# tensorflow/recommenders

Measured on NVIDIA H100. Metric: queries/sec brute-force top-K (1Mx64 candidates), higher is better.
Workload: dtype f32 (fp16 wgmma screening, fp32 accumulate + exact fp32 re-scoring)

## Files before the change

### recommenders_b200/csrc/rowselect.cuh

```cuda
#pragma once
#include "common.cuh"
#include <limits.h>

namespace tfrs {

constexpr int RS_THREADS = 256;

__device__ __forceinline__ void bitonic_sort_desc(float* bs, long long* bi, int P) {
  for (int size = 2; size <= P; size <<= 1) {
    for (int stride = size >> 1; stride > 0; stride >>= 1) {
      for (int t = threadIdx.x; t < (P >> 1); t += blockDim.x) {
        int lo = 2 * t - (t & (stride - 1));
        int hi = lo + stride;
        bool desc = ((lo & size) == 0);
        float sl = bs[lo], sh = bs[hi];
        long long il = bi[lo], ih = bi[hi];
        bool hi_better = better(sh, ih, sl, il);
        bool lo_better = better(sl, il, sh, ih);
        if (desc ? hi_better : lo_better) { bs[lo] = sh; bs[hi] = sl; bi[lo] = ih; bi[hi] = il; }
      }
      __syncthreads();
    }
  }
}

static inline int pow2_ceil(int x) { int p = 1; while (p < x) p <<= 1; return p; }
static inline int rowselect_cap(int k) { int c = pow2_ceil(2 * k); return c < 1024 ? 1024 : c; }
static inline size_t rowselect_smem(int cap, size_t extra) { return (size_t)cap * 12 + extra; }

template <class Provider>
__global__ void __launch_bounds__(RS_THREADS)
row_topk_kernel(Provider prov, int k, int cap, float* __restrict__ out_s, long long* __restrict__ out_i,
                int out_ld) {
  extern __shared__ __align__(16) unsigned char rs_smem[];
  long long* bi = reinterpret_cast<long long*>(rs_smem);
  float* bs = reinterpret_cast<float*>(rs_smem + (size_t)cap * 8);
  void* extra = rs_smem + (size_t)cap * 12;
  __shared__ int cnt_sh;
  __shared__ float thr_s_sh;
  __shared__ long long thr_i_sh;
  __shared__ int full_sh;

  const int row = blockIdx.x;
  const int tid = threadIdx.x;
  if (tid == 0) { cnt_sh = 0; full_sh = 0; thr_s_sh = 0.f; thr_i_sh = 0; }
  prov.begin(row, extra);
  __syncthreads();

  const long long total = prov.count(row);
  const int min_room = cap / 4;
  long long pos = 0;
  while (pos < total) {
    __syncthreads();
    const int cnt0 = cnt_sh;
    const bool full = full_sh != 0;
    const float ts = thr_s_sh;
    const long long ti = thr_i_sh;
    __syncthreads();
    const int slab = (int)min((long long)(cap - cnt0), total - pos);
    for (int t = tid; t < slab; t += RS_THREADS) {
      float s; long long i;
      prov.get(row, pos + t, s, i);
      if (!full || better(s, i, ts, ti)) {
        int p = atomicAdd(&cnt_sh, 1);
        bs[p] = s; bi[p] = i;
      }
    }
    __syncthreads();
    pos += slab;
    const int cnt = cnt_sh;
    if (pos < total && cap - cnt >= min_room) continue;
    int P = 2; while (P < cnt) P <<= 1;
    for (int t = cnt + tid; t < P; t += RS_THREADS) { bs[t] = -INFINITY; bi[t] = LLONG_MAX; }
    __syncthreads();
    if (cnt > 1) bitonic_sort_desc(bs, bi, P);
    if (tid == 0) {
      int keep = cnt < k ? cnt : k;
      cnt_sh = keep;
      if (keep == k) { full_sh = 1; thr_s_sh = bs[k - 1]; thr_i_sh = bi[k - 1]; }
    }
  }
  __syncthreads();
  const int n_out = cnt_sh;
  for (int t = tid; t < n_out; t += RS_THREADS) {
    out_s[(long long)row * out_ld + t] = bs[t];
    out_i[(long long)row * out_ld + t] = bi[t];
  }
}

}
```

### recommenders_b200/csrc/topk_tc.cu

```cuda
#include <cuda_fp16.h>
#include <math.h>
#include <stdlib.h>
#include <type_traits>
#include "rowselect.cuh"
#include "tc_ptx.cuh"

namespace tfrs {
namespace tc {

constexpr int TILE_N = 128;
constexpr int TILE_M = 128;
constexpr int QBLK = 256;
constexpr int KSLAB = 64;
constexpr int SLAB_BYTES = TILE_N * 128;
constexpr int HEADER_BYTES = 1024;
constexpr int THREADS = 512;
constexpr int CONSUMER_WARPS = 16;
constexpr int CAND_CAP = 2048;
constexpr int MAX_SAMPLE_STRIDE = 4;
constexpr int FIN_MAX_PARTS = 2 * 132;
constexpr int MAX_BINS = 1024;
constexpr int FP16_TARGET = 15;
constexpr float E_REL = 0.00108f;
constexpr float E_ACC = 0.00013f;
// ... 380 lines not shown
}
__device__ __forceinline__ unsigned int warp_kth_largest_smem(const unsigned int* keys, int n, int k, int lane, unsigned int prefix, int top_bit) {
  for (int bit = top_bit; bit >= 0; --bit) {
    const unsigned int cand = prefix | (1u << bit);
    int c = 0;
    for (int t = lane; t < n; t += 32) c += (keys[t] >= cand) ? 1 : 0;
    c = __reduce_add_sync(0xffffffffu, c);
    if (c >= k) prefix = cand;
  }
  return prefix;
}

template <int KPL>
__global__ void __launch_bounds__(256)
tc_threshold_kernel(const float* __restrict__ binmax, int bins_ld, int n_bins, int k, const float* __restrict__ margin,
                    float* __restrict__ thr, unsigned int* __restrict__ overflow, long long Q) {
  const int lane = threadIdx.x & 31;
  const long long row = ((long long)blockIdx.x * 256 + threadIdx.x) >> 5;
  if (row >= Q) return;
  const float* src = binmax + row * bins_ld;
  unsigned int key[KPL];
#pragma unroll
  for (int j = 0; j < KPL; ++j) { const int i = j * 32 + lane; key[j] = i < n_bins ? f2key(__ldg(src + i)) : 0u; }
  const unsigned int kth = warp_kth_largest_regs<KPL>(key, k);
  if (lane == 0) { thr[row] = key2f(kth) - margin[row]; overflow[row] = 0; }
}

enum { FIN_TOPK = 0, FIN_EXCLUDE = 1, FIN_COUNT = 2 };
constexpr int FW_WARPS = 4;

struct FinParams {
  const float* q; const float* corpus; int d; int k; long long index_offset; long long N; long long Q;
  const unsigned int* count; const float* cand_s; const unsigned int* cand_i; int segs; int cap_part;
  const float* cut; const float* thr; unsigned int* overflow;
  int cap_keys, cap_band;
  unsigned int* band_idx; int* band_n;
  int allow_short;
  float* out_s; long long* out_i;
  const long long* identifiers; const long long* exclusions; int n_excl; int k_out;
  const float* pos; const int* qexp; const IndexHeader* hdr; int* out_count;
};

__device__ __forceinline__ float exact_score(const float* __restrict__ qs, const float* __restrict__ c, int d) {
  float acc = 0.f;
  if ((d & 31) == 0) {
    for (int kk = 0; kk < d; kk += 32) {
      float4 cv[8];
#pragma unroll
      for (int u = 0; u < 8; ++u) cv[u] = __ldg(reinterpret_cast<const float4*>(c + kk) + u);
#pragma unroll
      for (int u = 0; u < 8; ++u) {
// ... 49 lines not shown
    akey[t] = ((unsigned long long)f2key(adj) << 32) | (unsigned long long)(0xFFFFFFFFu - (unsigned int)t);
  }
  __syncwarp();
  for (int t = lane; t < kf; t += 32) {
    const unsigned long long mine = akey[t];
    int rank = 0;
    for (int j = 0; j < kf; ++j) rank += (akey[j] > mine) ? 1 : 0;
    if (rank < p.k_out) {
      const unsigned long long e = srt[t];
      p.out_s[row * p.k_out + rank] = rank_key_score(e);
      p.out_i[row * p.k_out + rank] = (long long)rank_key_index(e) + p.index_offset;
    }
  }
}

__host__ __device__ inline size_t sel_warp_bytes(int cap_keys, int segs) {
  return (size_t)cap_keys * 4 + (size_t)cap_keys * 2 + (size_t)((segs + 1 + 3) & ~3) * 4;
}
constexpr int SEL_WARPS = 8;

__device__ __forceinline__ bool load_record(const FinParams& p, long long row, const int* soff, int rec, int total_rec,
                                            unsigned int& ix0, float (&sc)[8]) {
  if (rec >= total_rec) return false;
  int lo = 0, hi = p.segs;
  while (hi - lo > 1) { const int mid = (lo + hi) >> 1; if (soff[mid] <= rec) lo = mid; else hi = mid; }
  const long long at = (row * p.segs + lo) * p.cap_part + (rec - soff[lo]);
  ix0 = __ldg(p.cand_i + at);
  const float4 s0 = __ldg(reinterpret_cast<const float4*>(p.cand_s + at * 8));
  const float4 s1 = __ldg(reinterpret_cast<const float4*>(p.cand_s + at * 8) + 1);
  sc[0] = s0.x; sc[1] = s0.y; sc[2] = s0.z; sc[3] = s0.w; sc[4] = s1.x; sc[5] = s1.y; sc[6] = s1.z; sc[7] = s1.w;
  return true;
}

template <int MODE>
__global__ void __launch_bounds__(SEL_WARPS * 32)
tc_select_kernel(const FinParams p) {
  extern __shared__ __align__(16) unsigned char fsm[];
  const int warp = threadIdx.x >> 5, lane = threadIdx.x & 31;
  const long long row = (long long)blockIdx.x * SEL_WARPS + warp;
  if (row >= p.Q) return;
  unsigned char* base = fsm + (size_t)warp * sel_warp_bytes(p.cap_keys, p.segs);
  unsigned int* keys = reinterpret_cast<unsigned int*>(base);
  unsigned short* loc = reinterpret_cast<unsigned short*>(keys + p.cap_keys);
  int* soff = reinterpret_cast<int*>(loc + p.cap_keys);
  const unsigned int n32 = (unsigned int)p.N;
  unsigned int* band = p.band_idx + row * p.cap_band;

  int carry = 0; bool bad = false;
  for (int s0 = 0; s0 < p.segs; s0 += 32) {
    const int s = s0 + lane;
    int c = 0;
    if (s < p.segs) {
      const unsigned int cc = __ldg(p.count + row * p.segs + s);
      if (cc > (unsigned int)p.cap_part) bad = true; else c = (int)cc;
    }
    const int inc = warp_incl_scan(c, lane);
    if (s < p.segs) soff[s + 1] = carry + inc;
    carry += __shfl_sync(0xffffffffu, inc, 31);
  }
  if (lane == 0) soff[0] = 0;
  if (__any_sync(0xffffffffu, bad)) {
    if (lane == 0) { p.overflow[row] = 1; p.band_n[row] = 0; }
    return;
  }
  __syncwarp();
  const int total_rec = soff[p.segs];
  const float thr_row = p.thr[row];
  if (MODE != FIN_COUNT && total_rec >= 8192) {
    if (lane == 0) { p.overflow[row] = 1; p.band_n[row] = 0; }
    return;
  }

  if (MODE == FIN_COUNT) {
    const float eps = 0.5f * p.cut[row];
    const float pos_s = ldexpf(p.pos[row], p.hdr->st.exp + p.qexp[row]);
    const float hi = pos_s + eps, lo_b = pos_s - eps;
    int definite = 0, m = 0;
    for (int rb = 0; rb < total_rec; rb += 32) {
      unsigned int ix0 = 0, amb = 0; int cnt = 0; float sc[8];
      if (load_record(p, row, soff, rb + lane, total_rec, ix0, sc)) {
#pragma unroll
        for (int j = 0; j < 8; ++j) {
          const bool real = ix0 + j < n32;
          definite += (real && sc[j] > hi) ? 1 : 0;
          const bool a = real && sc[j] > lo_b && !(sc[j] > hi);
          amb |= a ? (1u << j) : 0u; cnt += a ? 1 : 0;
        }
      }
      const int incl = warp_incl_scan(cnt, lane);
      const int tot = __shfl_sync(0xffffffffu, incl, 31);
      if (m + tot <= p.cap_band) {
        int at_pos = m + incl - cnt;
#pragma unroll
        for (int j = 0; j < 8; ++j)
          if (amb & (1u << j)) { band[at_pos] = ix0 + j; ++at_pos; }
      }
      m += tot;
    }
    definite = __reduce_add_sync(0xffffffffu, definite);
    if (lane == 0) {
      if (definite >= p.k) { p.out_count[row] = p.k; p.band_n[row] = 0; p.overflow[row] = 0; }
      else if (m > p.cap_band) { p.overflow[row] = 1; p.band_n[row] = 0; }
      else { p.out_count[row] = definite; p.band_n[row] = m; p.overflow[row] = 0; }
    }
    return;
  }

  int n = 0;
  unsigned int kmax = 0u, kmin = 0xFFFFFFFFu;
  for (int rb = 0; rb < total_rec; rb += 32) {
    float sc[8]; unsigned int ix0 = 0, keep = 0; int cnt = 0;
    if (load_record(p, row, soff, rb + lane, total_rec, ix0, sc)) {
#pragma unroll
      for (int j = 0; j < 8; ++j) {
        const bool kp = sc[j] >= thr_row && ix0 + j < n32;
        keep |= kp ? (1u << j) : 0u; cnt += kp ? 1 : 0;
      }
    }
    const int incl = warp_incl_scan(cnt, lane);
    const int tot = __shfl_sync(0xffffffffu, incl, 31);
    if (n + tot <= p.cap_keys) {
      int at_pos = n + incl - cnt;
#pragma unroll
      for (int j = 0; j < 8; ++j) {
        if (keep & (1u << j)) {
          const unsigned int key = f2key(sc[j] + 0.0f);
          kmax = max(kmax, key); kmin = min(kmin, key);
          keys[at_pos] = key;
          loc[at_pos] = (unsigned short)(((rb + lane) << 3) | j);
          ++at_pos;
        }
      }
    }
    n += tot;
  }
  if (n > p.cap_keys || (n < p.k && !p.allow_short)) { if (lane == 0) { p.overflow[row] = 1; p.band_n[row] = 0; } return; }
  __syncwarp();
  if (n < p.k) {
    const bool fits = n <= p.cap_band;
    for (int t = lane; t < n && fits; t += 32) {
      const unsigned int l = loc[t];
      const int rec = (int)(l >> 3);
      int lo = 0, hi = p.segs;
      while (hi - lo > 1) { const int mid = (lo + hi) >> 1; if (soff[mid] <= rec) lo = mid; else hi = mid; }
      band[t] = __ldg(p.cand_i + (row * p.segs + lo) * p.cap_part + (rec - soff[lo])) + (l & 7u);
    }
    if (lane == 0) { p.overflow[row] = fits ? 0u : 1u; p.band_n[row] = fits ? n : 0; }
    return;
  }
  kmax = __reduce_max_sync(0xffffffffu, kmax); kmin = __reduce_min_sync(0xffffffffu, kmin);
  unsigned int tau_key;
  {
    const unsigned int diff = kmax ^ kmin;
    const int top = diff ? (31 - __clz(diff)) : -1;
    const unsigned int prefix0 = top >= 31 ? 0u : (top < 0 ? kmax : (kmax & ~((2u << top) - 1u)));
    if (n <= 512) {
      unsigned int kr[16];
#pragma unroll
      for (int j = 0; j < 16; ++j) { const int t = j * 32 + lane; kr[j] = t < n ? keys[t] : 0u; }
      tau_key = warp_kth_largest_regs<16>(kr, p.k, prefix0, top);
    } else if (n <= 1024) {
      unsigned int kr[32];
#pragma unroll
      for (int j = 0; j < 32; ++j) { const int t = j * 32 + lane; kr[j] = t < n ? keys[t] : 0u; }
      tau_key = warp_kth_largest_regs<32>(kr, p.k, prefix0, top);
    } else {
      tau_key = warp_kth_largest_smem(keys, n, p.k, lane, prefix0, top);
    }
  }
  const float lim = key2f(tau_key) - p.cut[row];
  if (!p.allow_short && (!(lim >= thr_row) || !(lim > -INFINITY))) { if (lane == 0) { p.overflow[row] = 1; p.band_n[row] = 0; } return; }
  const unsigned int lim_key = f2key(lim + 0.0f);
  const unsigned int lt_mask = (1u << lane) - 1u;
  int m = 0;
  for (int tb = 0; tb < n; tb += 32) {
    const int t = tb + lane;
    const bool kp = t < n && keys[t] >= lim_key;
    const unsigned int vote = __ballot_sync(0xffffffffu, kp);
    if (kp) {
      const int at_pos = m + __popc(vote & lt_mask);
      if (at_pos < p.cap_band) {
        const unsigned int l = loc[t];
        const int rec = (int)(l >> 3);
        int lo = 0, hi = p.segs;
        while (hi - lo > 1) { const int mid = (lo + hi) >> 1; if (soff[mid] <= rec) lo = mid; else hi = mid; }
        band[at_pos] = __ldg(p.cand_i + (row * p.segs + lo) * p.cap_part + (rec - soff[lo])) + (l & 7u);
      }
    }
    m += __popc(vote);
  }
  if (lane == 0) {
    if (m > p.cap_band) { p.overflow[row] = 1; p.band_n[row] = 0; }
    else { p.overflow[row] = 0; p.band_n[row] = m; }
  }
}

constexpr int RS_BLOCK = 128;
template <int MODE>
__global__ void __launch_bounds__(RS_BLOCK)
tc_rescore_kernel(const FinParams p) {
  extern __shared__ __align__(16) unsigned char rsm[];
  unsigned long long* sk = reinterpret_cast<unsigned long long*>(rsm);
  float* qs = reinterpret_cast<float*>(sk + p.cap_band);
  unsigned long long* srt = reinterpret_cast<unsigned long long*>(qs + ((p.d + 3) & ~3));
  __shared__ int greater_sh;
  const long long row = blockIdx.x;
  const int tid = threadIdx.x;
  if (p.overflow[row] != 0) return;
  const int m = p.band_n[row];
  if (MODE == FIN_COUNT && m == 0) return;
  for (int t = tid; t < p.d; t += RS_BLOCK) qs[t] = p.q[row * p.d + t];
  if (tid == 0) greater_sh = 0;
  __syncthreads();
  const unsigned int* band = p.band_idx + row * p.cap_band;
  if (MODE == FIN_COUNT) {
    const float pos = p.pos[row];
    int g = 0;
    for (int t = tid; t < m; t += RS_BLOCK) g += (exact_score(qs, p.corpus + (long long)band[t] * p.d, p.d) > pos) ? 1 : 0;
    g = __reduce_add_sync(0xffffffffu, g);
    if ((tid & 31) == 0 && g) atomicAdd(&greater_sh, g);
    __syncthreads();
    if (tid == 0) { const int c = p.out_count[row] + greater_sh; p.out_count[row] = c < p.k ? c : p.k; }
    return;
  }
  if (p.d == 64) {
    constexpr int RPB = RS_BLOCK / 8;
    constexpr int MAXR = 8;
    const int sub = tid & 7, grp = tid >> 3;
    for (int t0 = 0; t0 < m; t0 += RPB * MAXR) {
      float4 a[MAXR], b[MAXR];
#pragma unroll
      for (int r = 0; r < MAXR; ++r) {
        const int t = t0 + r * RPB + grp;
        if (t < m) {
          const float4* src = reinterpret_cast<const float4*>(p.corpus + (long long)band[t] * 64) + sub * 2;
          a[r] = __ldg(src); b[r] = __ldg(src + 1);
        }
      }
      const float q0 = qs[sub * 8], q1 = qs[sub * 8 + 1], q2 = qs[sub * 8 + 2], q3 = qs[sub * 8 + 3];
      const float q4 = qs[sub * 8 + 4], q5 = qs[sub * 8 + 5], q6 = qs[sub * 8 + 6], q7 = qs[sub * 8 + 7];
#pragma unroll
      for (int r = 0; r < MAXR; ++r) {
        const int t = t0 + r * RPB + grp;
        const bool live = t < m;
        float acc = 0.f;
#pragma unroll
        for (int step = 0; step < 8; ++step) {
          if (sub == step && live) {
            acc = fmaf(q0, a[r].x, acc); acc = fmaf(q1, a[r].y, acc); acc = fmaf(q2, a[r].z, acc); acc = fmaf(q3, a[r].w, acc);
            acc = fmaf(q4, b[r].x, acc); acc = fmaf(q5, b[r].y, acc); acc = fmaf(q6, b[r].z, acc); acc = fmaf(q7, b[r].w, acc);
          }
          acc = __shfl_sync(0xffffffffu, acc, (threadIdx.x & 24) | step);
        }
        if (live && sub == 0) sk[t] = rank_key(acc, band[t]);
      }
    }
  } else {
    for (int t = tid; t < m; t += RS_BLOCK) {
      const unsigned int idx = band[t];
      sk[t] = rank_key(exact_score(qs, p.corpus + (long long)idx * p.d, p.d), idx);
    }
  }
  __syncthreads();
  if (MODE == FIN_TOPK && m < p.k)
    for (int t = m + tid; t < p.k; t += RS_BLOCK) { p.out_s[row * p.k + t] = -INFINITY; p.out_i[row * p.k + t] = LLONG_MAX; }
  for (int t = tid; t < m; t += RS_BLOCK) {
    const unsigned long long mine = sk[t];
    int rank = 0;
#pragma unroll 4
    for (int j = 0; j < m; ++j) rank += (sk[j] > mine) ? 1 : 0;
    if (rank < p.k) {
      if (MODE == FIN_TOPK) {
        p.out_s[row * p.k + rank] = rank_key_score(mine);
        p.out_i[row * p.k + rank] = (long long)rank_key_index(mine) + p.index_offset;
      } else {
        srt[rank] = mine;
      }
    }
  }
  if (MODE == FIN_EXCLUDE) {
    __syncthreads();
// ... 22 lines not shown
  __device__ void begin(int row, void* extra) {
    qs = reinterpret_cast<float*>(extra);
    if (overflow[row] != 0) for (int t = threadIdx.x; t < d; t += blockDim.x) qs[t] = q[(long long)row * d + t];
  }
  __device__ long long count(int row) const { return overflow[row] != 0 ? N : 0; }
  __device__ void get(int, long long t, float& s, long long& i) const {
    const float* c = corpus + t * d;
    float acc = 0.f;
    for (int kk = 0; kk < d; ++kk) acc = fmaf(qs[kk], __ldg(c + kk), acc);
    s = acc; i = index_offset + t;
  }
};

__global__ void __launch_bounds__(256)
tc_count_fallback_kernel(const float* __restrict__ q, const float* __restrict__ corpus, long long N, int d, int k,
                         const float* __restrict__ pos, const unsigned int* __restrict__ overflow, int* __restrict__ out_count) {
  __shared__ float qs[128];
  __shared__ int total;
  const int row = blockIdx.x;
  if (overflow[row] == 0) return;
  for (int t = threadIdx.x; t < d; t += 256) qs[t] = q[(long long)row * d + t];
  if (threadIdx.x == 0) total = 0;
  __syncthreads();
  const float ps = pos[row];
  int c = 0;
  for (long long t = threadIdx.x; t < N; t += 256) {
    const float* cr = corpus + t * d;
    float acc = 0.f;
    for (int kk = 0; kk < d; ++kk) acc = fmaf(qs[kk], __ldg(cr + kk), acc);
    c += (acc + 0.0f > ps) ? 1 : 0;
  }
  c = __reduce_add_sync(0xffffffffu, c);
  if ((threadIdx.x & 31) == 0) atomicAdd(&total, c);
  __syncthreads();
  if (threadIdx.x == 0) out_count[row] = total < k ? total : k;
}

struct Prof {
  bool on = false;
  static constexpr int MAXC = 512, STAGES_ = 4;
  cudaEvent_t ev[MAXC][STAGES_ + 1];
  int created = 0, calls = 0;
};
static Prof g_prof;
static void prof_mark(cudaStream_t st, int stage) {
  if (!g_prof.on || g_prof.calls >= Prof::MAXC) return;
  int c = g_prof.calls;
  while (g_prof.created <= c) {
    for (int s = 0; s <= Prof::STAGES_; ++s) cudaEventCreate(&g_prof.ev[g_prof.created][s]);
    ++g_prof.created;
  }
  cudaEventRecord(g_prof.ev[c][stage], st);
  if (stage == Prof::STAGES_) ++g_prof.calls;
}

struct Plan {
  int kb, stages; long long n_tiles; int nqb; long long Qp;
  int stride, n_sample, group, bins_per_part, n_bins, bins_ld, parts_sample, parts_full, cap_part, cap_keys, cap_band;
  size_t smem;
  size_t o_qimg, o_margin, o_cut, o_thr, o_qexp, o_count, o_ovf, o_binmax, o_cand, o_tmp, o_band, o_bandn, total;
};

static bool make_plan(long long Q, long long N, int d, int k, Plan& pl) {
  if (d <= 0 || d > 128 || Q <= 0 || N <= 0 || k <= 0) return false;
  pl.kb = (d + KSLAB - 1) / KSLAB;
  pl.stages = pl.kb == 1 ? 6 : 4;
  pl.n_tiles = ceil_div(N, TILE_N);
  pl.nqb = (int)ceil_div(Q, QBLK);
  pl.Qp = (long long)pl.nqb * QBLK;
  if (k > 256 || N >= (1ll << 31)) return false;
  const long long full_tiles = N / TILE_N;
  if (full_tiles < 1) return false;
  pl.stride = MAX_SAMPLE_STRIDE;
#ifdef TFRS_DEBUG_SWITCHES
  { static int ov = getenv("TFRS_TC_SAMPLE_STRIDE") ? atoi(getenv("TFRS_TC_SAMPLE_STRIDE")) : 0; if (ov >= 1 && ov <= 16) pl.stride = ov; }
// ... 26 lines not shown
    pl.cap_band = ck / 2;
  }
  pl.smem = (size_t)(2 + pl.stages) * pl.kb * SLAB_BYTES + 1024  + 256 ;
  size_t o = 0;
  auto take = [&](size_t bytes) { size_t r = o; o += align_up(bytes, 1024); return r; };
  pl.o_qimg = take((size_t)pl.nqb * 2 * pl.kb * SLAB_BYTES);
  pl.o_margin = take((size_t)pl.Qp * 4);
  pl.o_cut = take((size_t)pl.Qp * 4);
  pl.o_thr = take((size_t)pl.Qp * 4);
  pl.o_qexp = take((size_t)pl.Qp * 4);
  pl.o_count = take((size_t)pl.Qp * pl.parts_full * 2 * 4);
  pl.o_ovf = take((size_t)pl.Qp * 4);
  pl.o_binmax = take((size_t)pl.Qp * pl.bins_ld * 4);
  pl.o_cand = take((size_t)pl.Qp * pl.parts_full * 2 * pl.cap_part * (8 * 4 + 4));
  pl.o_tmp = take((size_t)Q * k * 12);
  pl.o_band = take((size_t)pl.Qp * pl.cap_band * 4);
  pl.o_bandn = take((size_t)pl.Qp * 4);
  pl.total = o;
  return true;
}

template <int KB, int STAGES>
static int launch_scans(const Plan& pl, ScanParams sp, cudaStream_t st, int mode) {
  auto ks = tc_scan_kernel<KB, STAGES, MODE_SAMPLE>;
  auto kf = tc_scan_kernel<KB, STAGES, MODE_FILTER>;
  TFRS_DYN_SMEM(ks, (int)pl.smem);
  TFRS_DYN_SMEM(kf, (int)pl.smem);
  if (mode == MODE_SAMPLE) {
    sp.parts = pl.parts_sample; sp.n_seq = pl.n_sample; sp.stride = pl.stride;
    ks<<<(unsigned)(pl.nqb * sp.parts), THREADS, pl.smem, st>>>(sp);
  } else {
    sp.parts = pl.parts_full; sp.n_seq = (int)pl.n_tiles; sp.stride = 1;
    kf<<<(unsigned)(pl.nqb * sp.parts), THREADS, pl.smem, st>>>(sp);
  }
  TFRS_LAUNCH_CHECK();
  return TFRS_OK;
}

static int launch_scan_mode(const Plan& pl, const ScanParams& sp, cudaStream_t st, int mode) {
  if (pl.kb == 1) return launch_scans<1, 6>(pl, sp, st, mode);
  return launch_scans<2, 4>(pl, sp, st, mode);
}

template <int MODE>
static int launch_finalize(FinParams fp, cudaStream_t st) {
  auto ksel = tc_select_kernel<MODE>;
  auto krs = tc_rescore_kernel<MODE>;
  TFRS_DYN_SMEM(ksel, (int)(SEL_WARPS * sel_warp_bytes(4096, FIN_MAX_PARTS)));
  ksel<<<(unsigned)ceil_div(fp.Q, SEL_WARPS), SEL_WARPS * 32, SEL_WARPS * sel_warp_bytes(fp.cap_keys, fp.segs), st>>>(fp);
  TFRS_LAUNCH_CHECK();
  const size_t rs_smem = (size_t)fp.cap_band * 8 + (size_t)((fp.d + 3) & ~3) * 4 + (MODE == FIN_EXCLUDE ? (size_t)fp.k * 16 : 0);
  TFRS_DYN_SMEM(krs, 64 * 1024);
  krs<<<(unsigned)fp.Q, RS_BLOCK, rs_smem, st>>>(fp);
  TFRS_LAUNCH_CHECK();
  return TFRS_OK;
}

struct Call {
  int mode;
  const float* q; long long Q; const float* corpus; const void* index_buf; long long N; int d; int k; long long index_offset;
  void* ws; size_t ws_bytes; cudaStream_t st;
  float* out_s; long long* out_i;
  const long long* identifiers; const long long* exclusions; int n_excl; int k_out;
  const float* pos; int* out_count;
  ThrHook hook; void* hook_ctx; int allow_short;
};

static int run_call(const Call& c) {
// ... 6 lines not shown
  if (!c.ws || c.ws_bytes < pl.total + 16) { set_error("topk_tc: workspace too small (%zu < %zu)", c.ws_bytes, pl.total + 16); return TFRS_ERR_WORKSPACE_TOO_SMALL; }
  cudaStream_t st = c.st;
  unsigned char* w = (unsigned char*)(((uintptr_t)c.ws + 15) & ~(uintptr_t)15);
  unsigned char* qimg = w + pl.o_qimg;
  float* margin = (float*)(w + pl.o_margin);
  float* cut = (float*)(w + pl.o_cut);
  float* thr = (float*)(w + pl.o_thr);
  int* qexp = (int*)(w + pl.o_qexp);
  unsigned int* count = (unsigned int*)(w + pl.o_count);
  unsigned int* ovf = (unsigned int*)(w + pl.o_ovf);
  float* binmax = (float*)(w + pl.o_binmax);
  float* cand_s = (float*)(w + pl.o_cand);
  unsigned int* cand_i = (unsigned int*)(w + pl.o_cand + (size_t)pl.Qp * pl.parts_full * 2 * pl.cap_part * 32);
  float* tmp_s = (float*)(w + pl.o_tmp);
  long long* tmp_i = (long long*)(w + pl.o_tmp + align_up((size_t)c.Q * c.k * 4, 8));
  const IndexHeader* hdr = (const IndexHeader*)c.index_buf;
  const unsigned char* cimg = (const unsigned char*)c.index_buf + HEADER_BYTES;

  prof_mark(st, 0);
  tc_qprep_kernel<<<(unsigned)ceil_div(pl.Qp * 32, 256), 256, 0, st>>>(c.q, c.Q, pl.Qp, c.d, pl.kb, hdr, qimg, margin, cut, qexp);
  TFRS_LAUNCH_CHECK();
  ScanParams sp{};
  sp.qimg = qimg; sp.cimg = cimg; sp.Q = c.Q; sp.N = c.N; sp.nqb = pl.nqb; sp.n_tiles = pl.n_tiles;
  sp.binmax = binmax; sp.bins_ld = pl.bins_ld; sp.group = pl.group; sp.bins_per_part = pl.bins_per_part;
  sp.thr = thr; sp.count = count; sp.cand_s = cand_s; sp.cand_i = cand_i; sp.cap_part = pl.cap_part;
  prof_mark(st, 1);
  int rc = launch_scan_mode(pl, sp, st, MODE_SAMPLE);
  if (rc) return rc;
  if (pl.n_bins <= 512)
    tc_threshold_kernel<16><<<(unsigned)ceil_div(c.Q * 32, 256), 256, 0, st>>>(binmax, pl.bins_ld, pl.n_bins, c.k, margin, thr, ovf, c.Q);
  else
    tc_threshold_kernel<32><<<(unsigned)ceil_div(c.Q * 32, 256), 256, 0, st>>>(binmax, pl.bins_ld, pl.n_bins, c.k, margin, thr, ovf, c.Q);
  TFRS_LAUNCH_CHECK();
  if (c.hook) {
    rc = c.hook(c.hook_ctx, thr, margin, cut, qexp, &hdr->st.exp, c.Q, st);
    if (rc) return rc;
  }
  prof_mark(st, 2);
  rc = launch_scan_mode(pl, sp, st, MODE_FILTER);
  if (rc) return rc;
  prof_mark(st, 3);
  if (FILTER_ABLATION != FILTER_FULL) { prof_mark(st, 4); return TFRS_OK; }
  FinParams fp{};
  fp.q = c.q; fp.corpus = c.corpus; fp.d = c.d; fp.k = c.k; fp.index_offset = c.index_offset; fp.N = c.N; fp.Q = c.Q;
  fp.count = count; fp.cand_s = cand_s; fp.cand_i = cand_i; fp.segs = pl.parts_full * 2; fp.cap_part = pl.cap_part;
  fp.cut = cut; fp.thr = thr; fp.overflow = ovf; fp.out_s = c.out_s; fp.out_i = c.out_i;
  fp.cap_keys = pl.cap_keys; fp.cap_band = pl.cap_band; fp.allow_short = c.allow_short;
  fp.band_idx = (unsigned int*)(w + pl.o_band); fp.band_n = (int*)(w + pl.o_bandn);
  fp.identifiers = c.identifiers; fp.exclusions = c.exclusions; fp.n_excl = c.n_excl; fp.k_out = c.k_out;
  fp.pos = c.pos; fp.qexp = qexp; fp.hdr = hdr; fp.out_count = c.out_count;
  if (c.mode == FIN_TOPK) rc = launch_finalize<FIN_TOPK>(fp, st);
  else if (c.mode == FIN_EXCLUDE) rc = launch_finalize<FIN_EXCLUDE>(fp, st);
  else rc = launch_finalize<FIN_COUNT>(fp, st);
  if (rc) return rc;
  if (c.mode == FIN_COUNT) {
    tc_count_fallback_kernel<<<(unsigned)c.Q, 256, 0, st>>>(c.q, c.corpus, c.N, c.d, c.k, c.pos, ovf, c.out_count);
    TFRS_LAUNCH_CHECK();
  } else {
    FallbackProvider prov{c.q, c.corpus, c.N, c.d, c.index_offset, ovf, nullptr};
    int cap = rowselect_cap(c.k);
    TFRS_DYN_SMEM(row_topk_kernel<FallbackProvider>, 64 * 1024);
    float* fs = c.mode == FIN_TOPK ? c.out_s : tmp_s;
    long long* fi = c.mode == FIN_TOPK ? c.out_i : tmp_i;
    row_topk_kernel<FallbackProvider><<<(unsigned)c.Q, RS_THREADS, rowselect_smem(cap, (size_t)c.d * 4), st>>>(prov, c.k, cap, fs, fi, c.k);
    TFRS_LAUNCH_CHECK();
    if (c.mode == FIN_EXCLUDE) {
      tc_exclude_fallback_kernel<<<(unsigned)ceil_div(c.Q, FW_WARPS), FW_WARPS * 32, (size_t)FW_WARPS * 2 * c.k * 8, st>>>(fp, tmp_s, tmp_i, ovf);
      TFRS_LAUNCH_CHECK();
    }
  }
  prof_mark(st, 4);
  return TFRS_OK;
}

}
}

using namespace tfrs;
using namespace tfrs::tc;
// ... 117 lines not shown
```

Before: 2.409 million.

## Fuse select and rescore into one finalize kernel; compact fallback rows

The per-warp select kernel and the per-row rescore kernel become a single block-per-row finalize kernel. The candidate band now lives in shared memory rather than a global band buffer, which removes one launch and a global round trip. Rows that overflow are appended to a compact list, so the fallback kernels run a grid sized to occupancy over only those rows instead of launching one block per query that exits early. The cost is a larger shared-memory footprint per block and more block-level synchronisation during selection.

```diff
diff --git a/recommenders_b200/csrc/rowselect.cuh b/recommenders_b200/csrc/rowselect.cuh
--- a/recommenders_b200/csrc/rowselect.cuh
+++ b/recommenders_b200/csrc/rowselect.cuh
@@ -31,7 +31,7 @@
 template <class Provider>
 __global__ void __launch_bounds__(RS_THREADS)
 row_topk_kernel(Provider prov, int k, int cap, float* __restrict__ out_s, long long* __restrict__ out_i,
-                int out_ld) {
+                int out_ld, const int* __restrict__ list = nullptr, const unsigned int* __restrict__ list_n = nullptr) {
   extern __shared__ __align__(16) unsigned char rs_smem[];
   long long* bi = reinterpret_cast<long long*>(rs_smem);
   float* bs = reinterpret_cast<float*>(rs_smem + (size_t)cap * 8);
@@ -41,50 +41,54 @@
   __shared__ long long thr_i_sh;
   __shared__ int full_sh;
 
-  const int row = blockIdx.x;
   const int tid = threadIdx.x;
-  if (tid == 0) { cnt_sh = 0; full_sh = 0; thr_s_sh = 0.f; thr_i_sh = 0; }
-  prov.begin(row, extra);
-  __syncthreads();
+  const int n_rows = list ? (int)*list_n : (int)gridDim.x;
+  for (int b = blockIdx.x; b < n_rows; b += gridDim.x) {
+    const int row = list ? list[b] : b;
+    __syncthreads();
+    if (tid == 0) { cnt_sh = 0; full_sh = 0; thr_s_sh = 0.f; thr_i_sh = 0; }
+    prov.begin(row, extra);
+    __syncthreads();
 
-  const long long total = prov.count(row);
-  const int min_room = cap / 4;
-  long long pos = 0;
-  while (pos < total) {
-    __syncthreads();
-    const int cnt0 = cnt_sh;
-    const bool full = full_sh != 0;
-    const float ts = thr_s_sh;
-    const long long ti = thr_i_sh;
-    __syncthreads();
-    const int slab = (int)min((long long)(cap - cnt0), total - pos);
-    for (int t = tid; t < slab; t += RS_THREADS) {
-      float s; long long i;
-      prov.get(row, pos + t, s, i);
-      if (!full || better(s, i, ts, ti)) {
-        int p = atomicAdd(&cnt_sh, 1);
-        bs[p] = s; bi[p] = i;
+    const long long total = prov.count(row);
+    const int min_room = cap / 4;
+    long long pos = 0;
+    while (pos < total) {
+      __syncthreads();
+      const int cnt0 = cnt_sh;
+      const bool full = full_sh != 0;
+      const float ts = thr_s_sh;
+      const long long ti = thr_i_sh;
+      __syncthreads();
+      const int slab = (int)min((long long)(cap - cnt0), total - pos);
+      for (int t = tid; t < slab; t += RS_THREADS) {
+        float s; long long i;
+        prov.get(row, pos + t, s, i);
+        if (!full || better(s, i, ts, ti)) {
+          int p = atomicAdd(&cnt_sh, 1);
+          bs[p] = s; bi[p] = i;
+        }
+      }
+      __syncthreads();
+      pos += slab;
+      const int cnt = cnt_sh;
+      if (pos < total && cap - cnt >= min_room) continue;
+      int P = 2; while (P < cnt) P <<= 1;
+      for (int t = cnt + tid; t < P; t += RS_THREADS) { bs[t] = -INFINITY; bi[t] = LLONG_MAX; }
+      __syncthreads();
+      if (cnt > 1) bitonic_sort_desc(bs, bi, P);
+      if (tid == 0) {
+        int keep = cnt < k ? cnt : k;
+        cnt_sh = keep;
+        if (keep == k) { full_sh = 1; thr_s_sh = bs[k - 1]; thr_i_sh = bi[k - 1]; }
       }
     }
     __syncthreads();
-    pos += slab;
-    const int cnt = cnt_sh;
-    if (pos < total && cap - cnt >= min_room) continue;
-    int P = 2; while (P < cnt) P <<= 1;
-    for (int t = cnt + tid; t < P; t += RS_THREADS) { bs[t] = -INFINITY; bi[t] = LLONG_MAX; }
-    __syncthreads();
-    if (cnt > 1) bitonic_sort_desc(bs, bi, P);
-    if (tid == 0) {
-      int keep = cnt < k ? cnt : k;
-      cnt_sh = keep;
-      if (keep == k) { full_sh = 1; thr_s_sh = bs[k - 1]; thr_i_sh = bi[k - 1]; }
+    const int n_out = cnt_sh;
+    for (int t = tid; t < n_out; t += RS_THREADS) {
+      out_s[(long long)row * out_ld + t] = bs[t];
+      out_i[(long long)row * out_ld + t] = bi[t];
     }
-  }
-  __syncthreads();
-  const int n_out = cnt_sh;
-  for (int t = tid; t < n_out; t += RS_THREADS) {
-    out_s[(long long)row * out_ld + t] = bs[t];
-    out_i[(long long)row * out_ld + t] = bi[t];
   }
 }
 
diff --git a/recommenders_b200/csrc/topk_tc.cu b/recommenders_b200/csrc/topk_tc.cu
--- a/recommenders_b200/csrc/topk_tc.cu
+++ b/recommenders_b200/csrc/topk_tc.cu
@@ -418,10 +418,11 @@
 template <int KPL>
 __global__ void __launch_bounds__(256)
 tc_threshold_kernel(const float* __restrict__ binmax, int bins_ld, int n_bins, int k, const float* __restrict__ margin,
-                    float* __restrict__ thr, unsigned int* __restrict__ overflow, long long Q) {
+                    float* __restrict__ thr, unsigned int* __restrict__ overflow, unsigned int* __restrict__ fb_n, long long Q) {
   const int lane = threadIdx.x & 31;
   const long long row = ((long long)blockIdx.x * 256 + threadIdx.x) >> 5;
   if (row >= Q) return;
+  if (row == 0 && lane == 0) *fb_n = 0;
   const float* src = binmax + row * bins_ld;
   unsigned int key[KPL];
 #pragma unroll
@@ -438,7 +439,7 @@
   const unsigned int* count; const float* cand_s; const unsigned int* cand_i; int segs; int cap_part;
   const float* cut; const float* thr; unsigned int* overflow;
   int cap_keys, cap_band;
-  unsigned int* band_idx; int* band_n;
+  int* fb_rows; unsigned int* fb_n;
   int allow_short;
   float* out_s; long long* out_i;
   const long long* identifiers; const long long* exclusions; int n_excl; int k_out;
@@ -518,17 +519,26 @@
   }
 }
 
-__host__ __device__ inline size_t sel_warp_bytes(int cap_keys, int segs) {
-  return (size_t)cap_keys * 4 + (size_t)cap_keys * 2 + (size_t)((segs + 1 + 3) & ~3) * 4;
-}
-constexpr int SEL_WARPS = 8;
+constexpr int FIN_BLOCK = 128;
+constexpr int FIN_MIN_BLOCKS = 8;
+__host__ __device__ inline size_t fin_smem_bytes(int cap_keys, int cap_band, int segs, int d, int k, int mode) {
+  return (size_t)cap_keys * 6 + (size_t)cap_band * 4 + (size_t)((segs + 1 + 3) & ~3) * 4 + (size_t)((d + 3) & ~3) * 4 +
+         (mode == FIN_EXCLUDE ? (size_t)k * 16 : 0);
+}
+
+__device__ __forceinline__ long long record_at(const FinParams& p, long long row, const int* soff, int rec) {
+  int lo = 0, hi = p.segs;
+  while (hi - lo > 1) { const int mid = (lo + hi) >> 1; if (soff[mid] <= rec) lo = mid; else hi = mid; }
+  return (row * p.segs + lo) * p.cap_part + (rec - soff[lo]);
+}
+__device__ __forceinline__ unsigned int locator_index(const FinParams& p, long long row, const int* soff, unsigned int l) {
+  return __ldg(p.cand_i + record_at(p, row, soff, (int)(l >> 3))) + (l & 7u);
+}
 
 __device__ __forceinline__ bool load_record(const FinParams& p, long long row, const int* soff, int rec, int total_rec,
                                             unsigned int& ix0, float (&sc)[8]) {
   if (rec >= total_rec) return false;
-  int lo = 0, hi = p.segs;
-  while (hi - lo > 1) { const int mid = (lo + hi) >> 1; if (soff[mid] <= rec) lo = mid; else hi = mid; }
-  const long long at = (row * p.segs + lo) * p.cap_part + (rec - soff[lo]);
+  const long long at = record_at(p, row, soff, rec);
   ix0 = __ldg(p.cand_i + at);
   const float4 s0 = __ldg(reinterpret_cast<const float4*>(p.cand_s + at * 8));
   const float4 s1 = __ldg(reinterpret_cast<const float4*>(p.cand_s + at * 8) + 1);
@@ -536,51 +546,64 @@
   return true;
 }
 
+__device__ __forceinline__ int warp_append(int* counter, int tot, int lane) {
+  int base = 0;
+  if (lane == 0 && tot) base = atomicAdd(counter, tot);
+  return __shfl_sync(0xffffffffu, base, 0);
+}
+
+__device__ __forceinline__ void flag_fallback(const FinParams& p, long long row) {
+  p.overflow[row] = 1;
+  p.fb_rows[atomicAdd(p.fb_n, 1u)] = (int)row;
+}
+
 template <int MODE>
-__global__ void __launch_bounds__(SEL_WARPS * 32)
-tc_select_kernel(const FinParams p) {
+__global__ void __launch_bounds__(FIN_BLOCK, FIN_MIN_BLOCKS)
+tc_finalize_kernel(const FinParams p) {
   extern __shared__ __align__(16) unsigned char fsm[];
-  const int warp = threadIdx.x >> 5, lane = threadIdx.x & 31;
-  const long long row = (long long)blockIdx.x * SEL_WARPS + warp;
-  if (row >= p.Q) return;
-  unsigned char* base = fsm + (size_t)warp * sel_warp_bytes(p.cap_keys, p.segs);
-  unsigned int* keys = reinterpret_cast<unsigned int*>(base);
+  unsigned int* keys = reinterpret_cast<unsigned int*>(fsm);
   unsigned short* loc = reinterpret_cast<unsigned short*>(keys + p.cap_keys);
-  int* soff = reinterpret_cast<int*>(loc + p.cap_keys);
+  unsigned int* band = reinterpret_cast<unsigned int*>(loc + p.cap_keys);
+  int* soff = reinterpret_cast<int*>(band + p.cap_band);
+  float* qs = reinterpret_cast<float*>(soff + ((p.segs + 1 + 3) & ~3));
+  unsigned long long* srt = reinterpret_cast<unsigned long long*>(qs + ((p.d + 3) & ~3));
+  unsigned long long* sk = reinterpret_cast<unsigned long long*>(fsm);
+  __shared__ int n_sh, m_sh, definite_sh, greater_sh, bad_sh;
+  __shared__ unsigned int kmax_sh, kmin_sh, tau_sh;
+  const long long row = blockIdx.x;
+  const int tid = threadIdx.x, warp = tid >> 5, lane = tid & 31;
   const unsigned int n32 = (unsigned int)p.N;
-  unsigned int* band = p.band_idx + row * p.cap_band;
-
-  int carry = 0; bool bad = false;
-  for (int s0 = 0; s0 < p.segs; s0 += 32) {
-    const int s = s0 + lane;
-    int c = 0;
-    if (s < p.segs) {
-      const unsigned int cc = __ldg(p.count + row * p.segs + s);
-      if (cc > (unsigned int)p.cap_part) bad = true; else c = (int)cc;
-    }
-    const int inc = warp_incl_scan(c, lane);
-    if (s < p.segs) soff[s + 1] = carry + inc;
-    carry += __shfl_sync(0xffffffffu, inc, 31);
-  }
-  if (lane == 0) soff[0] = 0;
-  if (__any_sync(0xffffffffu, bad)) {
-    if (lane == 0) { p.overflow[row] = 1; p.band_n[row] = 0; }
-    return;
-  }
-  __syncwarp();
+
+  if (warp == 0) {
+    int carry = 0; bool bad = false;
+    for (int s0 = 0; s0 < p.segs; s0 += 32) {
+      const int s = s0 + lane;
+      int c = 0;
+      if (s < p.segs) {
+        const unsigned int cc = __ldg(p.count + row * p.segs + s);
+        if (cc > (unsigned int)p.cap_part) bad = true; else c = (int)cc;
+      }
+      const int inc = warp_incl_scan(c, lane);
+      if (s < p.segs) soff[s + 1] = carry + inc;
+      carry += __shfl_sync(0xffffffffu, inc, 31);
+    }
+    bad = __any_sync(0xffffffffu, bad);
+    if (lane == 0) {
+      soff[0] = 0; bad_sh = bad ? 1 : 0;
+      n_sh = 0; m_sh = 0; definite_sh = 0; greater_sh = 0; kmax_sh = 0u; kmin_sh = 0xFFFFFFFFu;
+    }
+  }
+  for (int t = tid; t < p.d; t += FIN_BLOCK) qs[t] = p.q[row * p.d + t];
+  __syncthreads();
   const int total_rec = soff[p.segs];
-  const float thr_row = p.thr[row];
-  if (MODE != FIN_COUNT && total_rec >= 8192) {
-    if (lane == 0) { p.overflow[row] = 1; p.band_n[row] = 0; }
-    return;
-  }
+  if (bad_sh || (MODE != FIN_COUNT && total_rec >= 8192)) { if (tid == 0) flag_fallback(p, row); return; }
 
   if (MODE == FIN_COUNT) {
     const float eps = 0.5f * p.cut[row];
     const float pos_s = ldexpf(p.pos[row], p.hdr->st.exp + p.qexp[row]);
     const float hi = pos_s + eps, lo_b = pos_s - eps;
-    int definite = 0, m = 0;
-    for (int rb = 0; rb < total_rec; rb += 32) {
+    int definite = 0;
+    for (int rb = warp * 32; rb < total_rec; rb += FIN_BLOCK) {
       unsigned int ix0 = 0, amb = 0; int cnt = 0; float sc[8];
       if (load_record(p, row, soff, rb + lane, total_rec, ix0, sc)) {
 #pragma unroll
@@ -593,143 +616,118 @@
       }
       const int incl = warp_incl_scan(cnt, lane);
       const int tot = __shfl_sync(0xffffffffu, incl, 31);
-      if (m + tot <= p.cap_band) {
-        int at_pos = m + incl - cnt;
+      const int base = warp_append(&m_sh, tot, lane);
+      if (base + tot <= p.cap_band) {
+        int at_pos = base + incl - cnt;
 #pragma unroll
         for (int j = 0; j < 8; ++j)
           if (amb & (1u << j)) { band[at_pos] = ix0 + j; ++at_pos; }
       }
-      m += tot;
     }
     definite = __reduce_add_sync(0xffffffffu, definite);
-    if (lane == 0) {
-      if (definite >= p.k) { p.out_count[row] = p.k; p.band_n[row] = 0; p.overflow[row] = 0; }
-      else if (m > p.cap_band) { p.overflow[row] = 1; p.band_n[row] = 0; }
-      else { p.out_count[row] = definite; p.band_n[row] = m; p.overflow[row] = 0; }
-    }
-    return;
-  }
-
-  int n = 0;
-  unsigned int kmax = 0u, kmin = 0xFFFFFFFFu;
-  for (int rb = 0; rb < total_rec; rb += 32) {
-    float sc[8]; unsigned int ix0 = 0, keep = 0; int cnt = 0;
-    if (load_record(p, row, soff, rb + lane, total_rec, ix0, sc)) {
-#pragma unroll
-      for (int j = 0; j < 8; ++j) {
-        const bool kp = sc[j] >= thr_row && ix0 + j < n32;
-        keep |= kp ? (1u << j) : 0u; cnt += kp ? 1 : 0;
-      }
-    }
-    const int incl = warp_incl_scan(cnt, lane);
-    const int tot = __shfl_sync(0xffffffffu, incl, 31);
-    if (n + tot <= p.cap_keys) {
-      int at_pos = n + incl - cnt;
-#pragma unroll
-      for (int j = 0; j < 8; ++j) {
-        if (keep & (1u << j)) {
-          const unsigned int key = f2key(sc[j] + 0.0f);
-          kmax = max(kmax, key); kmin = min(kmin, key);
-          keys[at_pos] = key;
-          loc[at_pos] = (unsigned short)(((rb + lane) << 3) | j);
-          ++at_pos;
-        }
-      }
-    }
-    n += tot;
-  }
-  if (n > p.cap_keys || (n < p.k && !p.allow_short)) { if (lane == 0) { p.overflow[row] = 1; p.band_n[row] = 0; } return; }
-  __syncwarp();
-  if (n < p.k) {
-    const bool fits = n <= p.cap_band;
-    for (int t = lane; t < n && fits; t += 32) {
-      const unsigned int l = loc[t];
-      const int rec = (int)(l >> 3);
-      int lo = 0, hi = p.segs;
-      while (hi - lo > 1) { const int mid = (lo + hi) >> 1; if (soff[mid] <= rec) lo = mid; else hi = mid; }
-      band[t] = __ldg(p.cand_i + (row * p.segs + lo) * p.cap_part + (rec - soff[lo])) + (l & 7u);
-    }
-    if (lane == 0) { p.overflow[row] = fits ? 0u : 1u; p.band_n[row] = fits ? n : 0; }
-    return;
-  }
-  kmax = __reduce_max_sync(0xffffffffu, kmax); kmin = __reduce_min_sync(0xffffffffu, kmin);
-  unsigned int tau_key;
-  {
-    const unsigned int diff = kmax ^ kmin;
-    const int top = diff ? (31 - __clz(diff)) : -1;
-    const unsigned int prefix0 = top >= 31 ? 0u : (top < 0 ? kmax : (kmax & ~((2u << top) - 1u)));
-    if (n <= 512) {
-      unsigned int kr[16];
-#pragma unroll
-      for (int j = 0; j < 16; ++j) { const int t = j * 32 + lane; kr[j] = t < n ? keys[t] : 0u; }
-      tau_key = warp_kth_largest_regs<16>(kr, p.k, prefix0, top);
-    } else if (n <= 1024) {
-      unsigned int kr[32];
-#pragma unroll
-      for (int j = 0; j < 32; ++j) { const int t = j * 32 + lane; kr[j] = t < n ? keys[t] : 0u; }
-      tau_key = warp_kth_largest_regs<32>(kr, p.k, prefix0, top);
-    } else {
-      tau_key = warp_kth_largest_smem(keys, n, p.k, lane, prefix0, top);
-    }
-  }
-  const float lim = key2f(tau_key) - p.cut[row];
-  if (!p.allow_short && (!(lim >= thr_row) || !(lim > -INFINITY))) { if (lane == 0) { p.overflow[row] = 1; p.band_n[row] = 0; } return; }
-  const unsigned int lim_key = f2key(lim + 0.0f);
-  const unsigned int lt_mask = (1u << lane) - 1u;
-  int m = 0;
-  for (int tb = 0; tb < n; tb += 32) {
-    const int t = tb + lane;
-    const bool kp = t < n && keys[t] >= lim_key;
-    const unsigned int vote = __ballot_sync(0xffffffffu, kp);
-    if (kp) {
-      const int at_pos = m + __popc(vote & lt_mask);
-      if (at_pos < p.cap_band) {
-        const unsigned int l = loc[t];
-        const int rec = (int)(l >> 3);
-        int lo = 0, hi = p.segs;
-        while (hi - lo > 1) { const int mid = (lo + hi) >> 1; if (soff[mid] <= rec) lo = mid; else hi = mid; }
-        band[at_pos] = __ldg(p.cand_i + (row * p.segs + lo) * p.cap_part + (rec - soff[lo])) + (l & 7u);
-      }
-    }
-    m += __popc(vote);
-  }
-  if (lane == 0) {
-    if (m > p.cap_band) { p.overflow[row] = 1; p.band_n[row] = 0; }
-    else { p.overflow[row] = 0; p.band_n[row] = m; }
-  }
-}
-
-constexpr int RS_BLOCK = 128;
-template <int MODE>
-__global__ void __launch_bounds__(RS_BLOCK)
-tc_rescore_kernel(const FinParams p) {
-  extern __shared__ __align__(16) unsigned char rsm[];
-  unsigned long long* sk = reinterpret_cast<unsigned long long*>(rsm);
-  float* qs = reinterpret_cast<float*>(sk + p.cap_band);
-  unsigned long long* srt = reinterpret_cast<unsigned long long*>(qs + ((p.d + 3) & ~3));
-  __shared__ int greater_sh;
-  const long long row = blockIdx.x;
-  const int tid = threadIdx.x;
-  if (p.overflow[row] != 0) return;
-  const int m = p.band_n[row];
-  if (MODE == FIN_COUNT && m == 0) return;
-  for (int t = tid; t < p.d; t += RS_BLOCK) qs[t] = p.q[row * p.d + t];
-  if (tid == 0) greater_sh = 0;
-  __syncthreads();
-  const unsigned int* band = p.band_idx + row * p.cap_band;
-  if (MODE == FIN_COUNT) {
+    if (lane == 0 && definite) atomicAdd(&definite_sh, definite);
+    __syncthreads();
+    const int m = m_sh;
+    definite = definite_sh;
+    if (definite >= p.k) { if (tid == 0) { p.out_count[row] = p.k; p.overflow[row] = 0; } return; }
+    if (m > p.cap_band) { if (tid == 0) flag_fallback(p, row); return; }
     const float pos = p.pos[row];
     int g = 0;
-    for (int t = tid; t < m; t += RS_BLOCK) g += (exact_score(qs, p.corpus + (long long)band[t] * p.d, p.d) > pos) ? 1 : 0;
+    for (int t = tid; t < m; t += FIN_BLOCK) g += (exact_score(qs, p.corpus + (long long)band[t] * p.d, p.d) > pos) ? 1 : 0;
     g = __reduce_add_sync(0xffffffffu, g);
-    if ((tid & 31) == 0 && g) atomicAdd(&greater_sh, g);
+    if (lane == 0 && g) atomicAdd(&greater_sh, g);
     __syncthreads();
-    if (tid == 0) { const int c = p.out_count[row] + greater_sh; p.out_count[row] = c < p.k ? c : p.k; }
+    if (tid == 0) { const int c = definite + greater_sh; p.out_count[row] = c < p.k ? c : p.k; p.overflow[row] = 0; }
     return;
   }
+
+  const float thr_row = p.thr[row];
+  {
+    unsigned int kmax = 0u, kmin = 0xFFFFFFFFu;
+    for (int rb = warp * 32; rb < total_rec; rb += FIN_BLOCK) {
+      float sc[8]; unsigned int ix0 = 0, keep = 0; int cnt = 0;
+      if (load_record(p, row, soff, rb + lane, total_rec, ix0, sc)) {
+#pragma unroll
+        for (int j = 0; j < 8; ++j) {
+          const bool kp = sc[j] >= thr_row && ix0 + j < n32;
+          keep |= kp ? (1u << j) : 0u; cnt += kp ? 1 : 0;
+        }
+      }
+      const int incl = warp_incl_scan(cnt, lane);
+      const int tot = __shfl_sync(0xffffffffu, incl, 31);
+      const int base = warp_append(&n_sh, tot, lane);
+      if (base + tot <= p.cap_keys) {
+        int at_pos = base + incl - cnt;
+#pragma unroll
+        for (int j = 0; j < 8; ++j) {
+          if (keep & (1u << j)) {
+            const unsigned int key = f2key(sc[j] + 0.0f);
+            kmax = max(kmax, key); kmin = min(kmin, key);
+            keys[at_pos] = key;
+            loc[at_pos] = (unsigned short)(((rb + lane) << 3) | j);
+            ++at_pos;
+          }
+        }
+      }
+    }
+    kmax = __reduce_max_sync(0xffffffffu, kmax); kmin = __reduce_min_sync(0xffffffffu, kmin);
+    if (lane == 0) { atomicMax(&kmax_sh, kmax); atomicMin(&kmin_sh, kmin); }
+  }
+  __syncthreads();
+  const int n = n_sh;
+  if (n > p.cap_keys || (n < p.k && !p.allow_short)) { if (tid == 0) flag_fallback(p, row); return; }
+  int m;
+  if (n < p.k) {
+    if (n > p.cap_band) { if (tid == 0) flag_fallback(p, row); return; }
+    for (int t = tid; t < n; t += FIN_BLOCK) band[t] = locator_index(p, row, soff, loc[t]);
+    m = n;
+  } else {
+    if (warp == 0) {
+      const unsigned int kmax = kmax_sh, kmin = kmin_sh;
+      const unsigned int diff = kmax ^ kmin;
+      const int top = diff ? (31 - __clz(diff)) : -1;
+      const unsigned int prefix0 = top >= 31 ? 0u : (top < 0 ? kmax : (kmax & ~((2u << top) - 1u)));
+      unsigned int tau_key;
+      if (n <= 512) {
+        unsigned int kr[16];
+#pragma unroll
+        for (int j = 0; j < 16; ++j) { const int t = j * 32 + lane; kr[j] = t < n ? keys[t] : 0u; }
+        tau_key = warp_kth_largest_regs<16>(kr, p.k, prefix0, top);
+      } else if (n <= 1024) {
+        unsigned int kr[32];
+#pragma unroll
+        for (int j = 0; j < 32; ++j) { const int t = j * 32 + lane; kr[j] = t < n ? keys[t] : 0u; }
+        tau_key = warp_kth_largest_regs<32>(kr, p.k, prefix0, top);
+      } else {
+        tau_key = warp_kth_largest_smem(keys, n, p.k, lane, prefix0, top);
+      }
+      if (lane == 0) tau_sh = tau_key;
+    }
+    __syncthreads();
+    const float lim = key2f(tau_sh) - p.cut[row];
+    if (!p.allow_short && (!(lim >= thr_row) || !(lim > -INFINITY))) { if (tid == 0) flag_fallback(p, row); return; }
+    const unsigned int lim_key = f2key(lim + 0.0f);
+    const unsigned int lt_mask = (1u << lane) - 1u;
+    for (int tb = warp * 32; tb < n; tb += FIN_BLOCK) {
+      const int t = tb + lane;
+      const bool kp = t < n && keys[t] >= lim_key;
+      const unsigned int vote = __ballot_sync(0xffffffffu, kp);
+      const int base = warp_append(&m_sh, __popc(vote), lane);
+      if (kp) {
+        const int at_pos = base + __popc(vote & lt_mask);
+        if (at_pos < p.cap_band) band[at_pos] = locator_index(p, row, soff, loc[t]);
+      }
+    }
+    __syncthreads();
+    m = m_sh;
+    if (m > p.cap_band) { if (tid == 0) flag_fallback(p, row); return; }
+  }
+  if (tid == 0) p.overflow[row] = 0;
+  __syncthreads();
+
   if (p.d == 64) {
-    constexpr int RPB = RS_BLOCK / 8;
-    constexpr int MAXR = 8;
+    constexpr int RPB = FIN_BLOCK / 8;
+    constexpr int MAXR = 4;
     const int sub = tid & 7, grp = tid >> 3;
     for (int t0 = 0; t0 < m; t0 += RPB * MAXR) {
       float4 a[MAXR], b[MAXR];
@@ -760,15 +758,15 @@
       }
     }
   } else {
-    for (int t = tid; t < m; t += RS_BLOCK) {
+    for (int t = tid; t < m; t += FIN_BLOCK) {
       const unsigned int idx = band[t];
       sk[t] = rank_key(exact_score(qs, p.corpus + (long long)idx * p.d, p.d), idx);
     }
   }
   __syncthreads();
   if (MODE == FIN_TOPK && m < p.k)
-    for (int t = m + tid; t < p.k; t += RS_BLOCK) { p.out_s[row * p.k + t] = -INFINITY; p.out_i[row * p.k + t] = LLONG_MAX; }
-  for (int t = tid; t < m; t += RS_BLOCK) {
+    for (int t = m + tid; t < p.k; t += FIN_BLOCK) { p.out_s[row * p.k + t] = -INFINITY; p.out_i[row * p.k + t] = LLONG_MAX; }
+  for (int t = tid; t < m; t += FIN_BLOCK) {
     const unsigned long long mine = sk[t];
     int rank = 0;
 #pragma unroll 4
@@ -821,26 +819,38 @@
 
 __global__ void __launch_bounds__(256)
 tc_count_fallback_kernel(const float* __restrict__ q, const float* __restrict__ corpus, long long N, int d, int k,
-                         const float* __restrict__ pos, const unsigned int* __restrict__ overflow, int* __restrict__ out_count) {
+                         const float* __restrict__ pos, const int* __restrict__ fb_rows, const unsigned int* __restrict__ fb_n,
+                         int* __restrict__ out_count) {
   __shared__ float qs[128];
   __shared__ int total;
-  const int row = blockIdx.x;
-  if (overflow[row] == 0) return;
-  for (int t = threadIdx.x; t < d; t += 256) qs[t] = q[(long long)row * d + t];
-  if (threadIdx.x == 0) total = 0;
-  __syncthreads();
-  const float ps = pos[row];
-  int c = 0;
-  for (long long t = threadIdx.x; t < N; t += 256) {
-    const float* cr = corpus + t * d;
-    float acc = 0.f;
-    for (int kk = 0; kk < d; ++kk) acc = fmaf(qs[kk], __ldg(cr + kk), acc);
-    c += (acc + 0.0f > ps) ? 1 : 0;
-  }
-  c = __reduce_add_sync(0xffffffffu, c);
-  if ((threadIdx.x & 31) == 0) atomicAdd(&total, c);
-  __syncthreads();
-  if (threadIdx.x == 0) out_count[row] = total < k ? total : k;
+  const int n_rows = (int)*fb_n;
+  for (int b = blockIdx.x; b < n_rows; b += gridDim.x) {
+    const int row = fb_rows[b];
+    __syncthreads();
+    for (int t = threadIdx.x; t < d; t += 256) qs[t] = q[(long long)row * d + t];
+    if (threadIdx.x == 0) total = 0;
+    __syncthreads();
+    const float ps = pos[row];
+    int c = 0;
+    for (long long t = threadIdx.x; t < N; t += 256) {
+      const float* cr = corpus + t * d;
+      float acc = 0.f;
+      for (int kk = 0; kk < d; ++kk) acc = fmaf(qs[kk], __ldg(cr + kk), acc);
+      c += (acc + 0.0f > ps) ? 1 : 0;
+    }
+    c = __reduce_add_sync(0xffffffffu, c);
+    if ((threadIdx.x & 31) == 0) atomicAdd(&total, c);
+    __syncthreads();
+    if (threadIdx.x == 0) out_count[row] = total < k ? total : k;
+  }
+}
+
+template <class K>
+static unsigned fallback_grid(K kernel, int threads, size_t smem, long long Q) {
+  int per_sm = 0;
+  if (cudaOccupancyMaxActiveBlocksPerMultiprocessor(&per_sm, kernel, threads, smem) != cudaSuccess || per_sm < 1) per_sm = 1;
+  const long long g = (long long)per_sm * sm_count();
+  return (unsigned)(g < Q ? g : Q);
 }
 
 struct Prof {
@@ -865,7 +875,7 @@
   int kb, stages; long long n_tiles; int nqb; long long Qp;
   int stride, n_sample, group, bins_per_part, n_bins, bins_ld, parts_sample, parts_full, cap_part, cap_keys, cap_band;
   size_t smem;
-  size_t o_qimg, o_margin, o_cut, o_thr, o_qexp, o_count, o_ovf, o_binmax, o_cand, o_tmp, o_band, o_bandn, total;
+  size_t o_qimg, o_margin, o_cut, o_thr, o_qexp, o_count, o_ovf, o_binmax, o_cand, o_tmp, o_fbrows, o_fbn, total;
 };
 
 static bool make_plan(long long Q, long long N, int d, int k, Plan& pl) {
@@ -922,8 +932,8 @@
   pl.o_binmax = take((size_t)pl.Qp * pl.bins_ld * 4);
   pl.o_cand = take((size_t)pl.Qp * pl.parts_full * 2 * pl.cap_part * (8 * 4 + 4));
   pl.o_tmp = take((size_t)Q * k * 12);
-  pl.o_band = take((size_t)pl.Qp * pl.cap_band * 4);
-  pl.o_bandn = take((size_t)pl.Qp * 4);
+  pl.o_fbrows = take((size_t)Q * 4);
+  pl.o_fbn = take(4);
   pl.total = o;
   return true;
 }
@@ -952,14 +962,9 @@
 
 template <int MODE>
 static int launch_finalize(FinParams fp, cudaStream_t st) {
-  auto ksel = tc_select_kernel<MODE>;
-  auto krs = tc_rescore_kernel<MODE>;
-  TFRS_DYN_SMEM(ksel, (int)(SEL_WARPS * sel_warp_bytes(4096, FIN_MAX_PARTS)));
-  ksel<<<(unsigned)ceil_div(fp.Q, SEL_WARPS), SEL_WARPS * 32, SEL_WARPS * sel_warp_bytes(fp.cap_keys, fp.segs), st>>>(fp);
-  TFRS_LAUNCH_CHECK();
-  const size_t rs_smem = (size_t)fp.cap_band * 8 + (size_t)((fp.d + 3) & ~3) * 4 + (MODE == FIN_EXCLUDE ? (size_t)fp.k * 16 : 0);
-  TFRS_DYN_SMEM(krs, 64 * 1024);
-  krs<<<(unsigned)fp.Q, RS_BLOCK, rs_smem, st>>>(fp);
+  auto kfin = tc_finalize_kernel<MODE>;
+  TFRS_DYN_SMEM(kfin, (int)fin_smem_bytes(4096, 2048, FIN_MAX_PARTS, 128, 256, MODE));
+  kfin<<<(unsigned)fp.Q, FIN_BLOCK, fin_smem_bytes(fp.cap_keys, fp.cap_band, fp.segs, fp.d, fp.k, MODE), st>>>(fp);
   TFRS_LAUNCH_CHECK();
   return TFRS_OK;
 }
@@ -996,6 +1001,8 @@
   unsigned int* cand_i = (unsigned int*)(w + pl.o_cand + (size_t)pl.Qp * pl.parts_full * 2 * pl.cap_part * 32);
   float* tmp_s = (float*)(w + pl.o_tmp);
   long long* tmp_i = (long long*)(w + pl.o_tmp + align_up((size_t)c.Q * c.k * 4, 8));
+  int* fb_rows = (int*)(w + pl.o_fbrows);
+  unsigned int* fb_n = (unsigned int*)(w + pl.o_fbn);
   const IndexHeader* hdr = (const IndexHeader*)c.index_buf;
   const unsigned char* cimg = (const unsigned char*)c.index_buf + HEADER_BYTES;
 
@@ -1010,9 +1017,9 @@
   int rc = launch_scan_mode(pl, sp, st, MODE_SAMPLE);
   if (rc) return rc;
   if (pl.n_bins <= 512)
-    tc_threshold_kernel<16><<<(unsigned)ceil_div(c.Q * 32, 256), 256, 0, st>>>(binmax, pl.bins_ld, pl.n_bins, c.k, margin, thr, ovf, c.Q);
+    tc_threshold_kernel<16><<<(unsigned)ceil_div(c.Q * 32, 256), 256, 0, st>>>(binmax, pl.bins_ld, pl.n_bins, c.k, margin, thr, ovf, fb_n, c.Q);
   else
-    tc_threshold_kernel<32><<<(unsigned)ceil_div(c.Q * 32, 256), 256, 0, st>>>(binmax, pl.bins_ld, pl.n_bins, c.k, margin, thr, ovf, c.Q);
+    tc_threshold_kernel<32><<<(unsigned)ceil_div(c.Q * 32, 256), 256, 0, st>>>(binmax, pl.bins_ld, pl.n_bins, c.k, margin, thr, ovf, fb_n, c.Q);
   TFRS_LAUNCH_CHECK();
   if (c.hook) {
     rc = c.hook(c.hook_ctx, thr, margin, cut, qexp, &hdr->st.exp, c.Q, st);
@@ -1028,7 +1035,7 @@
   fp.count = count; fp.cand_s = cand_s; fp.cand_i = cand_i; fp.segs = pl.parts_full * 2; fp.cap_part = pl.cap_part;
   fp.cut = cut; fp.thr = thr; fp.overflow = ovf; fp.out_s = c.out_s; fp.out_i = c.out_i;
   fp.cap_keys = pl.cap_keys; fp.cap_band = pl.cap_band; fp.allow_short = c.allow_short;
-  fp.band_idx = (unsigned int*)(w + pl.o_band); fp.band_n = (int*)(w + pl.o_bandn);
+  fp.fb_rows = fb_rows; fp.fb_n = fb_n;
   fp.identifiers = c.identifiers; fp.exclusions = c.exclusions; fp.n_excl = c.n_excl; fp.k_out = c.k_out;
   fp.pos = c.pos; fp.qexp = qexp; fp.hdr = hdr; fp.out_count = c.out_count;
   if (c.mode == FIN_TOPK) rc = launch_finalize<FIN_TOPK>(fp, st);
@@ -1036,15 +1043,18 @@
   else rc = launch_finalize<FIN_COUNT>(fp, st);
   if (rc) return rc;
   if (c.mode == FIN_COUNT) {
-    tc_count_fallback_kernel<<<(unsigned)c.Q, 256, 0, st>>>(c.q, c.corpus, c.N, c.d, c.k, c.pos, ovf, c.out_count);
+    tc_count_fallback_kernel<<<fallback_grid(tc_count_fallback_kernel, 256, 0, c.Q), 256, 0, st>>>(
+        c.q, c.corpus, c.N, c.d, c.k, c.pos, fb_rows, fb_n, c.out_count);
     TFRS_LAUNCH_CHECK();
   } else {
     FallbackProvider prov{c.q, c.corpus, c.N, c.d, c.index_offset, ovf, nullptr};
     int cap = rowselect_cap(c.k);
-    TFRS_DYN_SMEM(row_topk_kernel<FallbackProvider>, 64 * 1024);
+    auto kfb = row_topk_kernel<FallbackProvider>;
+    TFRS_DYN_SMEM(kfb, 64 * 1024);
     float* fs = c.mode == FIN_TOPK ? c.out_s : tmp_s;
     long long* fi = c.mode == FIN_TOPK ? c.out_i : tmp_i;
-    row_topk_kernel<FallbackProvider><<<(unsigned)c.Q, RS_THREADS, rowselect_smem(cap, (size_t)c.d * 4), st>>>(prov, c.k, cap, fs, fi, c.k);
+    const size_t fb_smem = rowselect_smem(cap, (size_t)c.d * 4);
+    kfb<<<fallback_grid(kfb, RS_THREADS, fb_smem, c.Q), RS_THREADS, fb_smem, st>>>(prov, c.k, cap, fs, fi, c.k, fb_rows, fb_n);
     TFRS_LAUNCH_CHECK();
     if (c.mode == FIN_EXCLUDE) {
       tc_exclude_fallback_kernel<<<(unsigned)ceil_div(c.Q, FW_WARPS), FW_WARPS * 32, (size_t)FW_WARPS * 2 * c.k * 8, st>>>(fp, tmp_s, tmp_i, ovf);
```

Measured after the change: 2.458 million (median of 6 runs). +2.0%, better.
